# 42jaylonw/shifu

Measured on AMD Instinct MI355X. Metric: env-steps/sec (whole node), A1 12-dof 4096 envs/GPU, higher is better.
Workload: dtype f32

## Files before the change

shifu_amd/csrc/shf_a1_chain.hip:

```cpp
#include <hip/hip_runtime.h>

#include "shf_chain.h"
#include "shf_chain_hard.h"

template <int G, bool TW, bool SELF = false>
__global__ __launch_bounds__(256, (G == 32 ? 2 : 1)) void k_a1_chain(A1Args A) { a1_chain_step_body<G, A1Chain, TW, SELF>(A); }

#ifndef SHF_WR_FUSED
#define SHF_WR_FUSED 8
#endif
#ifndef SHF_WR_HOOK
#define SHF_WR_HOOK 0
#endif
template <bool TW, bool SELF>
__global__ __launch_bounds__(256, 2) void k_a1_chain_pgs(A1Args A) { a1_chain_step_body<32, A1Chain, TW, SELF, true, 8, false, SHF_WR_FUSED>(A); }
template <bool TW, bool SELF>
__global__ __launch_bounds__(256, 2) void k_a1_chain_pgs16(A1Args A) { a1_chain_step_body<32, A1Chain, TW, SELF, true, 16>(A); }
template <bool TW, bool SELF>
__global__ __launch_bounds__(256, 2) void k_a1_chain_tgs(A1Args A) { a1_chain_step_body<32, A1Chain, TW, SELF, true, 8, true, SHF_WR_FUSED>(A); }
template <bool TW, bool SELF>
__global__ __launch_bounds__(256, 2) void k_a1_chain_tgs16(A1Args A) { a1_chain_step_body<32, A1Chain, TW, SELF, true, 16, true>(A); }
#define SHF_PICK4(K, warped, self) ((self) ? ((warped) ? reinterpret_cast<const void*>(K<true, true>) : reinterpret_cast<const void*>(K<false, true>)) \
                                           : ((warped) ? reinterpret_cast<const void*>(K<true, false>) : reinterpret_cast<const void*>(K<false, false>)))
const void* shf_a1_chain_pgs_kernel(bool warped, bool self, bool k16, bool tgs) {
  if (tgs) return k16 ? SHF_PICK4(k_a1_chain_tgs16, warped, self) : SHF_PICK4(k_a1_chain_tgs, warped, self);
  return k16 ? SHF_PICK4(k_a1_chain_pgs16, warped, self) : SHF_PICK4(k_a1_chain_pgs, warped, self);
}
int shf_a1_chain_pgs_max_contacts(void) { return 16; }

template <bool TW, bool SELF, int KC, bool TGS>
DEV void sim_step_chain_pgs_body(const SimArgs& A) {
  extern __shared__ __attribute__((aligned(16))) float smem[];
  typedef A1Chain CD;
  constexpr int G = 32, nb = CD::NB, nd = CD::ND, NR = (CD::NEV + G - 1) / G;
  const int es = threadIdx.x / G, l = threadIdx.x % G;
  const int e = blockIdx.x * (256 / G) + es;
  stage_block<CHAIN_MODEL_BYTES>(A.model, smem);
  __syncthreads();
  const ShfModel* m = reinterpret_cast<const ShfModel*>(smem);
  if (e >= A.n) return;
  ChainLds L = chain_lds_carve<CD>(smem + CHAIN_MODEL_WORDS + es * chain_lds_words<CD>(0, SELF));
  const float* dof = A.dof + (size_t)e * nd * 2;
  const float* root = A.root + (size_t)e * 13;
  for (int i = l; i < 2 * nd; i += G) L.dofb[(i >> 1) * DOF_STRIDE + (i & 1)] = dof[i];
  if (l < 13) L.root[l] = root[l];
  GROUP_SYNC();
  StepCtx C;
  C.m = m; C.sp = A.sp; C.terr.t = A.terr; C.terr.h = A.heights; C.scene = nullptr;
  C.dropped = env_dropped(A.dropped, A.sp, e);
  C.mscale = A.mscale ? A.mscale + (size_t)e * nb : nullptr;
  const float mu = A.friction ? A.friction[e] : 1.0f;
  const int dl = l < nd ? l : 0;
  DofLane X = {L.dofb[dl * DOF_STRIDE], L.dofb[dl * DOF_STRIDE + 1], (A.effort && l < nd) ? A.effort[(size_t)e * nd + l] : 0.0f,
               (A.pos_tgt && l < nd) ? A.pos_tgt[(size_t)e * nd + l] : 0.0f, (A.vel_tgt && l < nd) ? A.vel_tgt[(size_t)e * nd + l] : 0.0f};
  ChainPoints<NR> LP;
  chain_points_load<G>(m, CD::NEV, l, C.sp.contact_offset + C.sp.rest_offset, LP);
  const RowLane RL = row_lane_load<CD>(l);
  chain_substep_hard<G, CD, TW, SELF, KC, TGS, (KC == 8 ? SHF_WR_HOOK : 0)>(C, L, l, X, LP, RL, A.body_force ? A.body_force + (size_t)e * nb * 3 : nullptr, mu, L.xch);
  if (l < nd) {
    A.dof[((size_t)e * nd + l) * 2] = X.q;
    A.dof[((size_t)e * nd + l) * 2 + 1] = X.qd;
  }
  if (l < 13) A.root[(size_t)e * 13 + l] = L.root[l];
  for (int i = l; i < 3 * nb; i += G) A.contact[(size_t)e * nb * 3 + i] = L.xch[i];
}
template <bool TW, bool SELF>
__global__ __launch_bounds__(256, 2) void k_sim_step_chain_pgs(SimArgs A) { sim_step_chain_pgs_body<TW, SELF, 8, false>(A); }
template <bool TW, bool SELF>
__global__ __launch_bounds__(256, 2) void k_sim_step_chain_pgs16(SimArgs A) { sim_step_chain_pgs_body<TW, SELF, 16, false>(A); }
template <bool TW, bool SELF>
__global__ __launch_bounds__(256, 2) void k_sim_step_chain_tgs(SimArgs A) { sim_step_chain_pgs_body<TW, SELF, 8, true>(A); }
template <bool TW, bool SELF>
__global__ __launch_bounds__(256, 2) void k_sim_step_chain_tgs16(SimArgs A) { sim_step_chain_pgs_body<TW, SELF, 16, true>(A); }
const void* shf_sim_step_chain_pgs_kernel(bool warped, bool self, bool k16, bool tgs) {
  if (tgs) return k16 ? SHF_PICK4(k_sim_step_chain_tgs16, warped, self) : SHF_PICK4(k_sim_step_chain_tgs, warped, self);
  return k16 ? SHF_PICK4(k_sim_step_chain_pgs16, warped, self) : SHF_PICK4(k_sim_step_chain_pgs, warped, self);
}
size_t shf_sim_step_chain_pgs_lds_bytes(bool self) { return ((size_t)CHAIN_MODEL_WORDS + 8 * (size_t)chain_lds_words<A1Chain>(0, self)) * 4; }

bool shf_a1_chain_matches(const ShfModel& m) { return A1Chain::matches(m); }
size_t shf_a1_chain_lds_bytes(int G, int nobs, bool self) {
  const int epb = 256 / G;
  return ((size_t)CHAIN_MODEL_WORDS + TASK_WORDS + STATS_LDS_WORDS + (size_t)epb * chain_lds_words<A1Chain>(SCR_OBS + nobs, self)) * 4;
}
const void* shf_a1_chain_kernel(int G, bool warped, bool self) {
  if (self) {
    if (G != 32) return nullptr;
    return warped ? reinterpret_cast<const void*>(k_a1_chain<32, true, true>) : reinterpret_cast<const void*>(k_a1_chain<32, false, true>);
  }
  switch (G) {
    case 16: return warped ? reinterpret_cast<const void*>(k_a1_chain<16, true>) : reinterpret_cast<const void*>(k_a1_chain<16, false>);
    case 32: return warped ? reinterpret_cast<const void*>(k_a1_chain<32, true>) : reinterpret_cast<const void*>(k_a1_chain<32, false>);
    default: return nullptr;
  }
}
#ifdef SHF_PHASE_CLOCK
int shf_a1_chain_phase_cycles(unsigned long long* out, int n, int reset) {
  unsigned long long h[48];
  if (hipMemcpyFromSymbol(h, HIP_SYMBOL(g_phase_cycles), sizeof h) != hipSuccess) return 1;
  for (int k = 0; k < n && k < 48; k++) out[k] = h[k];
  if (reset) {
    unsigned long long z[48] = {};
    if (hipMemcpyToSymbol(HIP_SYMBOL(g_phase_cycles), z, sizeof z) != hipSuccess) return 1;
  }
  return 0;
}
int shf_a1_chain_phase_waves(unsigned long long* out, int reset) {
  if (hipMemcpyFromSymbol(out, HIP_SYMBOL(g_phase_wave), sizeof(g_phase_wave)) != hipSuccess) return 1;
  if (reset) {
    void* p = nullptr;
    if (hipGetSymbolAddress(&p, HIP_SYMBOL(g_phase_wave)) != hipSuccess || hipMemset(p, 0, sizeof(g_phase_wave)) != hipSuccess) return 1;
// ... 5 lines not shown
```

shifu_amd/csrc/shf_chain.h:

```cpp
#pragma once
#include "shf_task.h"
#include "shf_link.h"

template <int NCH_, int NLK_, int NP_, int NEV_>
struct ChainDims {
  static constexpr int NCH = NCH_, NLK = NLK_, NB = 1 + NCH_ * (NLK_ + 1), ND = NCH_ * NLK_, NPC = NP_;
  static constexpr int NEV = NEV_;
  static constexpr int MAXPT = 9;
  static_assert(NEV_ >= NP_ && NEV_ <= 128, "evaluation slots: two 64-bit ballot words");
  DEV static constexpr int body(int c, int k) { return 1 + c * (NLK_ + 1) + k; }
  static bool matches(const ShfModel& m) {
    if (m.nb != NB || m.nd != ND || m.np != NPC || m.fixed_base || m.jtype[0] != SHF_JOINT_ROOT) return false;
    if (m.child_count[0] != NCH || m.nlevels != NLK) return false;
    if ((m.neval > 0 ? m.neval : m.np) != NEV) return false;
    int occupied = 0;
    for (int s = 0; s < NEV; s++) {
      const int i = m.pt_eval[s];
      if (i == -1) continue;
      if (i < 0 || i >= NPC || m.pt_slot[i] != s) return false;
      occupied++;
    }
    if (occupied != NPC) return false;
    for (int b = 0; b < NB; b++) {
      const int n = m.pt_count[b], i0 = m.pt_start[b];
      if (n > MAXPT) return false;
      if (n == 0 || m.dyn[b] != b) continue;
      const int s0 = m.pt_slot[i0];
      for (int j = 0; j < n; j++)
        if (m.pt_slot[i0 + j] != s0 + j) return false;
      if ((s0 >> 5) != ((s0 + n - 1) >> 5)) return false;
    }
    for (int c = 0; c < NCH; c++) {
      if (m.child_list[m.child_start[0] + c] != 1 + c * (NLK + 1)) return false;
      for (int k = 0; k <= NLK; k++) {
        const int b = 1 + c * (NLK + 1) + k;
        if (m.parent[b] != (k == 0 ? 0 : b - 1)) return false;
        if (k < NLK) {
          if (m.jtype[b] != SHF_JOINT_REVOLUTE || m.dof[b] != c * NLK + k || m.dyn[b] != b || m.level[b] != k + 1) return false;
          if (m.child_count[b] != (k < NLK - 1 ? 1 : 0)) return false;
          if (k < NLK - 1 && m.child_list[m.child_start[b]] != b + 1) return false;
        } else {
          if (m.jtype[b] != SHF_JOINT_WELD || m.dyn[b] != b - 1 || m.dof[b] != -1) return false;
        }
      }
    }
    return true;
  }
};
typedef ChainDims<4, 3, 76, 88> A1Chain;

#define JREC_STRIDE 16
#define JREC_QD 9
#define JREC_T0 12
#define JREC_DE 13
#define JREC_S 0
#define JREC_C 6
#define CHAIN_MODEL_BYTES ((int)offsetof(ShfModel, link_collide))
#define CHAIN_MODEL_WORDS ((CHAIN_MODEL_BYTES / 4 + 3) & ~3)
static_assert(CHAIN_MODEL_BYTES % 16 == 0, "stage_block copies 16-byte words");
template <class CD>
__host__ __device__ inline int chain_lds_words(int min_tail, bool self = false) {
  int tail = (CD::NPC + (self ? SHF_MAX_SELF_CONTACTS : 0)) * PT_STRIDE;
  if (tail < min_tail) tail = min_tail;
  const int w = CD::NB * POSE_STRIDE + ((CD::NB * 6 + 3) & ~3) + (CD::ND + 1) * XCH_STRIDE + CD::ND * JREC_STRIDE +
                ((CD::ND * DOF_STRIDE + 3) & ~3) + root_words(1) + tail;
  return (w + 3) & ~3;
}
struct ChainLds : EnvLds {
  float* jrec;
  float* xroot;
};
template <class CD>
DEV ChainLds chain_lds_carve(float* base) {
  static_assert(CD::ND * XCH_STRIDE >= 3 * CD::NB, "the exchange slots double as the contact-force staging");
  ChainLds L;
  L.pose = base;
  L.acc = L.pose + CD::NB * POSE_STRIDE;
  L.xch = L.acc + ((CD::NB * 6 + 3) & ~3);
  L.xroot = L.xch + CD::ND * XCH_STRIDE;
  L.jrec = L.xroot + XCH_STRIDE;
  L.dofb = L.jrec + CD::ND * JREC_STRIDE;
  L.root = L.dofb + ((CD::ND * DOF_STRIDE + 3) & ~3);
  L.pt = L.root + root_words(1);
  return L;
}

DEV void chain_ext_force(const float* F, const float* com, const float* Rw, const float* p, float* pA) {
  if (F[0] == 0.0f && F[1] == 0.0f && F[2] == 0.0f) return;
  float cw[3], t[3];
  mv3(Rw, com, cw);
#pragma unroll
  for (int k = 0; k < 3; k++) cw[k] += p[k];
  cross3(cw, F, t);
#pragma unroll
  for (int k = 0; k < 3; k++) { pA[k] -= t[k]; pA[3 + k] -= F[k]; }
}

DEV void chain_dof_effort(const StepCtx& C, int d, float q, float qd, float tau_cmd, float* t0o, float* deo, float tq = 0.0f, float tv_in = 0.0f) {
  const ShfModel* m = C.m;
  const float dt = C.sp.dt;
  float t0 = 0.0f, de = m->armature[d];
  const int mode = m->drive_mode[d];
  if (mode == SHF_DOF_MODE_EFFORT) {
    t0 = tau_cmd;
  } else if (mode == SHF_DOF_MODE_POS || mode == SHF_DOF_MODE_VEL) {
    float kp = mode == SHF_DOF_MODE_POS ? m->kp[d] : 0.0f, kd = m->kd[d];
    const float tv = mode == SHF_DOF_MODE_VEL ? tv_in : 0.0f;
    const float est = fmaf(kp, tq - q, kd * (tv - qd));
    const float lim = m->effort[d];
    if (lim > 0.0f && fabsf(est) > lim) { const float sc = lim / fabsf(est); kp *= sc; kd *= sc; }
    const float bj = fmaf(dt, kp, kd);
    t0 = fmaf(kp, tq - q, fmaf(kd, tv, -(bj * qd)));
    de = fmaf(dt, bj, de);
  }
  const float jd = m->damping[d];
  if (jd > 0.0f) { t0 = fmaf(-jd, qd, t0); de = fmaf(dt, jd, de); }
  const float lo = m->lower[d], up = m->upper[d];
  const float viol = q < lo ? lo - q : (q > up ? up - q : 0.0f);
  if (viol != 0.0f) {
    const float bl = fmaf(dt, C.sp.limit_k, C.sp.limit_d);
    t0 = fmaf(C.sp.limit_k, viol, fmaf(-bl, qd, t0));
    de = fmaf(dt, bl, de);
  }
  *t0o = t0; *deo = de;
}

template <int NR>
struct ChainPoints {
  int idx[NR];
  int body[NR];
  float pos[NR][3], rad[NR], thr[NR];
};
template <int G, int NR>
DEV void chain_points_load(const ShfModel* m, int nev, int l, float offset, ChainPoints<NR>& P) {
#pragma unroll
  for (int k = 0; k < NR; k++) {
    const int s = l + k * G;
    const int e = s < nev ? m->pt_eval[s] : -1;
    const int i = e < 0 ? 0 : e;
    P.idx[k] = e;
    P.body[k] = m->pt_body[i];
    P.rad[k] = m->pt_radius[i];
    P.thr[k] = (offset + P.rad[k]) * 1.01f + 1e-6f;
#pragma unroll
    for (int j = 0; j < 3; j++) P.pos[k][j] = m->pt_pos[i][j];
  }
}

DEV void terrain_height_gradient(const TerrainDev& T, float x, float y, float* h, float* gxo, float* gyo) {
  if (T.t.rows == 0) { *h = 0.0f; *gxo = 0.0f; *gyo = 0.0f; return; }
  float inv = 1.0f / T.t.hscale;
  float fx = (x + T.t.border) * inv, fy = (y + T.t.border) * inv;
  float fi = rclampf(floorf(fx), 0.0f, (float)(T.t.rows - 2)), fj = rclampf(floorf(fy), 0.0f, (float)(T.t.cols - 2));
  int i = (int)fi, j = (int)fj;
  float u = rclampf(fx - fi, 0.0f, 1.0f), v = rclampf(fy - fj, 0.0f, 1.0f);
  float vs = T.t.vscale;
  const int16_t* row0 = T.h + (size_t)i * T.t.cols + j;
  const int16_t* row1 = row0 + T.t.cols;
  float h00 = (float)row0[0] * vs, h10 = (float)row1[0] * vs, h01 = (float)row0[1] * vs, h11 = (float)row1[1] * vs;
  const bool lo = u + v <= 1.0f;
  float gx = (lo ? h10 : h11) - (lo ? h00 : h01);
  float gy = (lo ? h01 : h11) - (lo ? h00 : h10);
  *h = fmaf(lo ? v : 1.0f - v, lo ? gy : -gy, fmaf(lo ? u : 1.0f - u, lo ? gx : -gx, lo ? h00 : h11));
  *gxo = gx * inv; *gyo = gy * inv;
}
DEV void terrain_normal_from_gradient(const TerrainDev& T, float gx, float gy, float* n) {
  if (T.t.rows == 0) { n[0] = 0.0f; n[1] = 0.0f; n[2] = 1.0f; return; }
  const float nz = rsqrt_spec(fmaf(gy, gy, fmaf(gx, gx, 1.0f)));
  n[0] = -gx * nz; n[1] = -gy * nz; n[2] = nz;
}

struct SlotBits {
  unsigned long long w[2];
  DEV bool test(int s) const { return ((s < 64 ? w[0] >> s : w[1] >> (s - 64)) & 1ull) != 0ull; }
  DEV unsigned field(int s0, int n) const {
    const unsigned long long ww = s0 < 64 ? w[0] : w[1];
    return (unsigned)(ww >> (s0 & 63)) & ((1u << n) - 1u);
  }
};
template <int MAXPT>
struct SlotList {
  unsigned long long list;
  int i0, n, s0;
  SlotBits mask;
  DEV int slot(int j) const { return (int)((list >> (7 * j)) & 127ull); }
};
template <int MAXPT>
DEV SlotList<MAXPT> slot_list_load(const ShfModel* m, int i0, int n) {
  static_assert(MAXPT * 7 <= 64, "packed slot list");
  SlotList<MAXPT> S;
  S.list = 0ull; S.i0 = i0; S.n = n; S.s0 = m->pt_slot[n > 0 ? i0 : 0]; S.mask.w[0] = 0ull; S.mask.w[1] = 0ull;
  int sl[MAXPT];
#pragma unroll
  for (int j = 0; j < MAXPT; j++) sl[j] = m->pt_slot[j < n ? i0 + j : 0];
#pragma unroll
  for (int j = 0; j < MAXPT; j++) {
    if (j < n) {
      const int s = sl[j];
      S.list |= (unsigned long long)s << (7 * j);
      if (s < 64) S.mask.w[0] |= 1ull << s; else S.mask.w[1] |= 1ull << (s - 64);
    }
  }
  return S;
}

struct DofLane {
  float q, qd, tau;
  float tq, tv;
};

struct RowLane {
  int c, i;
  bool on;
  int off[6];
};
template <class CD>
DEV RowLane row_lane_load(int l) {
// ... 52 lines not shown
    for (int k = 0; k < 3; k++) { vc[k] = L.root[10 + k]; vc[3 + k] = L.root[7 + k]; }
    if (isroot && !(ROWS && ischain)) {
      pose_store(L.pose, Rc, pc, vc);
    } else {
      const int b0 = CD::body(ci, 0);
#pragma unroll
      for (int k = 0; k < NLK; k++) {
        const int b = b0 + k;
        float* rec = L.jrec + (ci * NLK + k) * JREC_STRIDE;
        float Rl[9];
#pragma unroll
        for (int j = 0; j < 9; j++) Rl[j] = rec[j];
        if constexpr (ROWS) {
          float Sx[6], cx[6];
          chain_compose_link(m->tpos[b], m->axis[b], Rl, rec[JREC_QD], Rc, pc, vc, Sx, cx);
#pragma unroll
          for (int j = 0; j < 6; j++) { rec[JREC_S + j] = Sx[j]; rec[JREC_C + j] = cx[j]; }
        } else {
          chain_compose_link(m->tpos[b], m->axis[b], Rl, rec[JREC_QD], Rc, pc, vc, K[k].S, K[k].c);
        }
        pose_store(L.pose + b * POSE_STRIDE, Rc, pc, vc);
      }
      const int b = b0 + NLK;
      chain_kin_weld(m->tpos[b], m->trot[b], Rc, pc);
      pose_store(L.pose + b * POSE_STRIDE, Rc, pc, vc);
    }
  }
  GROUP_SYNC();
  PHASE_MARK(1);

  float IA[21], pA[6];
  if (isbody) {
    const float* pb = L.pose + myb * POSE_STRIDE;
    float Rb[9], pp[3], vb[6];
#pragma unroll
    for (int k = 0; k < 9; k++) Rb[k] = pb[k];
#pragma unroll
    for (int k = 0; k < 3; k++) pp[k] = pb[9 + k];
#pragma unroll
    for (int k = 0; k < 6; k++) vb[k] = pb[12 + k];
    {
      float mass = m->mass[myb], I6[6];
#pragma unroll
      for (int k = 0; k < 6; k++) I6[k] = m->inertia[myb][k];
      if (C.mscale) {
        const float s = C.mscale[myb];
        mass *= s;
#pragma unroll
        for (int k = 0; k < 6; k++) I6[k] *= s;
      }
      rigid_inertia_p(mass, m->com[myb], I6, Rb, pp, vb, IA, pA);
    }
    if (fext) {
      const float F[3] = {fext[3 * myb], fext[3 * myb + 1], fext[3 * myb + 2]};
      chain_ext_force(F, m->com[myb], Rb, pp, pA);
      if (islink && (lb % NLK) == NLK - 1) {
        const int bw = myb + 1;
        const float* pw = L.pose + bw * POSE_STRIDE;
        float Rw[9], pq[3];
#pragma unroll
        for (int k = 0; k < 9; k++) Rw[k] = pw[k];
#pragma unroll
        for (int k = 0; k < 3; k++) pq[k] = pw[9 + k];
        const float Fw[3] = {fext[3 * bw], fext[3 * bw + 1], fext[3 * bw + 2]};
        chain_ext_force(Fw, m->com[bw], Rw, pq, pA);
      }
    }
  }
  PHASE_MARK(2);

  const float kc = C.sp.contact_k, dc = C.sp.contact_d, veps = C.sp.friction_vel;
  const float beta = fmaf(kc, dt, dc);
  const float mu = 0.5f * (mu_shape + C.terr.t.friction);
  const ContactConsts KC = {dt, {g[0], g[1], g[2]}, kc, beta, mu, veps, C.sp.max_depen_vel, C.sp.contact_offset};
  SlotBits act = {{0ull, 0ull}};
  {
    float r[NR][3], gx[NR], gy[NR], dz[NR], n[3];
    bool near[NR];
    const float nzmin = TW ? 0.0f : C.terr.t.nz_min;
#pragma unroll
    for (int k = 0; k < NR; k++) {
      const float* pb = L.pose + P.body[k] * POSE_STRIDE;
      float Rb[9], h = 0.0f;
#pragma unroll
      for (int j = 0; j < 9; j++) Rb[j] = pb[j];
      mv3(Rb, P.pos[k], r[k]);
#pragma unroll
      for (int j = 0; j < 3; j++) r[k][j] += pb[9 + j];
      if constexpr (TW) {
        gx[k] = 0.0f; gy[k] = 0.0f; dz[k] = 0.0f;
        near[k] = P.idx[k] >= 0;
      } else {
        terrain_height_gradient(C.terr, L.root[0] + r[k][0], L.root[1] + r[k][1], &h, &gx[k], &gy[k]);
        dz[k] = L.root[2] + r[k][2] - h;
        near[k] = P.idx[k] >= 0 && !(dz[k] * nzmin >= P.thr[k]);
      }
    }
    const int lane0 = (int)(threadIdx.x & 63u) - l;
#pragma unroll
    for (int k = 0; k < NR; k++) {
      if (__ballot(near[k]) == 0ull) continue;
      float on = 0.0f;
      if (near[k]) {
        float phi;
        if constexpr (TW) {
          float h;
          terrain_query<true>(C.terr, L.root[0] + r[k][0], L.root[1] + r[k][1], &h, n);
          phi = fmaf(L.root[2] + r[k][2] - h, n[2], -P.rad[k]);
        } else {
          terrain_normal_from_gradient(C.terr, gx[k], gy[k], n);
          phi = fmaf(dz[k], n[2], -P.rad[k]);
        }
        if (phi < KC.offset)
          on = contact_point_response(KC, L.pose + P.body[k] * POSE_STRIDE, r[k], n, P.rad[k], phi, L.pt + P.idx[k] * PT_STRIDE);
      }
      const unsigned long long bits = (__ballot(on != 0.0f) >> lane0) & (G >= 64 ? ~0ull : ((1ull << (G & 63)) - 1ull));
      if (k * G < 64) act.w[0] |= bits << ((k * G) & 63); else act.w[1] |= bits << ((k * G - 64) & 63);
    }
  }
  int nself = 0;
  if constexpr (SELF) nself = self_contacts_eval<G>(C, L, l, CD::NPC, mu_shape);
  GROUP_SYNC();
  PHASE_MARK(3);

  if (isbody) {
    if constexpr (SPLIT) {
      unsigned bits = act.field(mine.s0, mine.n);
      while (bits) {
        const int j = __builtin_ctz(bits);
        bits &= bits - 1u;
        const float* o = L.pt + (mine.i0 + j) * PT_STRIDE;
        if (half == 0) contact_accumulate_half<0>(o, dt, IA, pA);
        else contact_accumulate_half<1>(o, dt, IA, pA);
      }
    } else if (((act.w[0] & mine.mask.w[0]) | (act.w[1] & mine.mask.w[1])) != 0ull) {
      for (int j = 0; j < mine.n; j++) {
        if (!act.test(mine.slot(j))) continue;
        contact_accumulate_p(L.pt + (mine.i0 + j) * PT_STRIDE, dt, IA, pA);
      }
    }
    if constexpr (SELF) {
      for (int k = 0; k < nself; k++) {
        const float* o = L.pt + (CD::NPC + k) * PT_STRIDE;
        const int p = (int)o[PT_ON] - 1;
        const int da = m->dyn[m->cap_body[m->pair_a[p]]], db = m->dyn[m->cap_body[m->pair_b[p]]];
        if (da != myb && db != myb) continue;
        const float ma = body_mass(C, da), mb = body_mass(C, db);
// ... 259 lines not shown
    joint_local_rotation(m->trot[b], m->axis[b], X.q, Rl);
#pragma unroll
    for (int k = 0; k < 9; k++) rec[k] = Rl[k];
    rec[9] = X.qd;
  }
  GROUP_SYNC();
  if (l < NCH || l == ND) {
    float Rc[9], pc[3] = {0.0f, 0.0f, 0.0f}, vc[6], S[6], c[6];
    quat_to_mat(L.root + 3, Rc);
#pragma unroll
    for (int k = 0; k < 3; k++) { vc[k] = L.root[10 + k]; vc[3 + k] = L.root[7 + k]; }
    if (l == ND) {
      pose_store(L.pose, Rc, pc, vc);
    } else {
      const int b0 = CD::body(l, 0);
#pragma unroll
      for (int k = 0; k < NLK; k++) {
        const float* rec = L.jrec + (l * NLK + k) * JREC_STRIDE;
        float Rl[9];
#pragma unroll
        for (int j = 0; j < 9; j++) Rl[j] = rec[j];
        chain_compose_link(m->tpos[b0 + k], m->axis[b0 + k], Rl, rec[9], Rc, pc, vc, S, c);
        pose_store(L.pose + (b0 + k) * POSE_STRIDE, Rc, pc, vc);
      }
      chain_kin_weld(m->tpos[b0 + NLK], m->trot[b0 + NLK], Rc, pc);
      pose_store(L.pose + (b0 + NLK) * POSE_STRIDE, Rc, pc, vc);
    }
  }
  GROUP_SYNC();
  for (int b = l; b < NB; b += G) {
    const float* pb = L.pose + b * POSE_STRIDE;
    float Rw[9], pp[3], v[6], t[3], q[4];
#pragma unroll
    for (int k = 0; k < 9; k++) Rw[k] = pb[k];
#pragma unroll
    for (int k = 0; k < 3; k++) pp[k] = pb[9 + k];
#pragma unroll
    for (int k = 0; k < 6; k++) v[k] = pb[12 + k];
    float* o = stage + 13 * b;
#pragma unroll
    for (int k = 0; k < 3; k++) o[k] = L.root[k] + pp[k];
    mat_to_quat(Rw, q);
#pragma unroll
    for (int k = 0; k < 4; k++) o[3 + k] = q[k];
    cross3(v, pp, t);
#pragma unroll
    for (int k = 0; k < 3; k++) { o[7 + k] = v[3 + k] + t[k]; o[10 + k] = v[k]; }
  }
  GROUP_SYNC();
}

template <int G, class CD, bool TW, bool SELF, int KC, bool TGS, int WR>
DEV void chain_substep_hard(const StepCtx& C, const ChainLds& L, int l, DofLane& X, const ChainPoints<(CD::NEV + G - 1) / G>& P,
                            const RowLane& RL, const float* fext, float mu_shape, float* contact_out);
template <int G, class CD, bool TW, bool SELF = false, bool HARD = false, int KC = 8, bool TGS = false, int WR = 0>
DEV void a1_chain_step_body(const A1Args& A) {
  extern __shared__ __attribute__((aligned(16))) float smem[];
  constexpr int NLK = CD::NLK, nb = CD::NB, nd = CD::ND, NR = (CD::NEV + G - 1) / G;
  PHASE_BEGIN();
  float* stats_lds = smem + CHAIN_MODEL_WORDS + TASK_WORDS;
  stats_block_init(stats_lds);
  const unsigned long long stats_step = stats_step_load(A.stats);
  const int epb = 256 / G, es = threadIdx.x / G, l = threadIdx.x % G;
  const int e = blockIdx.x * epb + es;
  const int n = A.S.n;
  constexpr int NW = (2 * nd + G - 1) / G;
  float pre_dof[NW], pre_root = 0.0f, pre_act = 0.0f;
#pragma unroll
  for (int k = 0; k < NW; k++) pre_dof[k] = 0.0f;
  static_assert(G >= 13 && G > nd, "one root word and one action per lane");
  if (e < n) {
#pragma unroll
    for (int k = 0; k < NW; k++)
      if (l + k * G < 2 * nd) pre_dof[k] = A.S.dof[(size_t)e * nd * 2 + l + k * G];
    if (l < 13) pre_root = A.S.root[(size_t)e * 13 + l];
    if (l < nd) pre_act = raw_action(A, e, l, nd, stats_step);
  }
  stage_block<(int)sizeof(ShfA1TaskParams)>(A.tp, smem + CHAIN_MODEL_WORDS);
  stage_block<CHAIN_MODEL_BYTES>(A.S.model, smem);
  __syncthreads();
  const ShfModel* m = reinterpret_cast<const ShfModel*>(smem);
  const ShfA1TaskParams& tp = *reinterpret_cast<const ShfA1TaskParams*>(smem + CHAIN_MODEL_WORDS);
  if (e >= n) return;
  const int H = tp.num_history, P = tp.num_height_points;
  const int nobs = 12 + 2 * nd + nd * H + P;
  const int env_words = chain_lds_words<CD>(SCR_OBS + nobs, SELF);
  ChainLds L = chain_lds_carve<CD>(smem + CHAIN_MODEL_WORDS + TASK_WORDS + STATS_LDS_WORDS + es * env_words);
  float* scr = L.pt;

#pragma unroll
  for (int k = 0; k < NW; k++) {
    const int i = l + k * G;
    if (i < 2 * nd) L.dofb[(i >> 1) * DOF_STRIDE + (i & 1)] = pre_dof[k];
  }
  if (l < 13) L.root[l] = pre_root;
  float act = 0.0f;
  if (l < nd) {
    act = rclampf(pre_act * tp.action_scale, -tp.clip_actions, tp.clip_actions);
    A.actions[(size_t)e * nd + l] = act;
  }
  GROUP_SYNC();

  if (l == 0) {
    const float gv[3] = {0.0f, 0.0f, -1.0f};
    float pg[3], blv[3], bav[3];
    quat_rotate_inverse(L.root + 3, L.root + 7, blv);
    quat_rotate_inverse(L.root + 3, L.root + 10, bav);
    quat_rotate_inverse(L.root + 3, gv, pg);
    float* o = A.base_vel + (size_t)e * 9;
#pragma unroll
    for (int k = 0; k < 3; k++) { o[k] = blv[k]; o[3 + k] = bav[k]; o[6 + k] = pg[k]; }
  }

  StepCtx C;
  C.m = m; C.sp = A.S.sp; C.terr.t = A.S.terr; C.terr.h = A.S.heights; C.scene = nullptr;
  if constexpr (HARD) C.dropped = env_dropped(A.S.dropped, A.S.sp, e);
  C.mscale = A.S.mscale ? A.S.mscale + (size_t)e * nb : nullptr;
  const float mu = A.S.friction[e];
  const int nsub = tp.decimation + (tp.extra_substep ? 1 : 0);
  const int dl = l < nd ? l : 0;
  DofLane X = {L.dofb[dl * DOF_STRIDE], L.dofb[dl * DOF_STRIDE + 1], 0.0f};
  const float pg_ = tp.p_gain[dl], dg_ = tp.d_gain[dl], q0_ = tp.default_dof_pos[dl], lim_ = m->effort[dl];
  ChainPoints<NR> LP;
  if constexpr (!(HARD && WR > 0)) chain_points_load<G>(m, CD::NEV, l, HARD ? C.sp.contact_offset + C.sp.rest_offset : C.sp.contact_offset, LP);
  const int lb = G >= 32 ? (l & 15) : l;
  const int mb = lb < nd ? CD::body(lb / NLK, lb % NLK) : 0;
  const SlotList<CD::MAXPT> mine = slot_list_load<CD::MAXPT>(m, m->pt_start[mb], (lb <= nd && l < 32) ? m->pt_count[mb] : 0);
  const RowLane RL = row_lane_load<CD>(l);
  PHASE_MARK(11);
  for (int it = 0; it < nsub; it++) {
    if (it < tp.decimation) {
      const float t = pg_ * (act + q0_ - X.q) - dg_ * X.qd;
      X.tau = rclampf(t, -lim_, lim_);
    }
    if constexpr (HARD)
      chain_substep_hard<G, CD, TW, SELF, KC, TGS, WR>(C, L, l, X, LP, RL, (it == tp.decimation) ? A.push + (size_t)e * nb * 3 : nullptr, mu,
                                    (it == nsub - 1) ? L.xch : nullptr);
    else
      chain_substep<G, CD, TW, SELF>(C, L, l, X, LP, mine, RL, (it == tp.decimation) ? A.push + (size_t)e * nb * 3 : nullptr, mu,
                                     (it == nsub - 1) ? L.xch : nullptr);
  }
  PHASE_RESET();
  if (l < nd) {
    float* D = L.dofb + l * DOF_STRIDE;
    D[0] = X.q; D[1] = X.qd; D[5] = X.tau;
    A.torques[(size_t)e * nd + l] = X.tau;
    scr[SCR_ACT + l] = act;
  }
  for (int i = l; i < 3 * nb; i += G) A.S.contact[(size_t)e * nb * 3 + i] = L.xch[i];
  for (int i = l; i < nd * H; i += G) scr[SCR_HIST + i] = A.history[(size_t)e * nd * H + i];
  PHASE_MARK(12);
  chain_body_states<G, CD>(m, L, l, X, scr + SCR_BODY);
  for (int i = l; i < 13 * nb; i += G) A.body_state[(size_t)e * nb * 13 + i] = scr[SCR_BODY + i];
  PHASE_RESET();
  a1_post_step<G>(A, m, tp, L, scr, e, l, stats_lds, stats_step);
}
```

shifu_amd/csrc/shf_chain_hard.h:

```cpp
#pragma once
#include "shf_chain.h"

#define UF_STRIDE 8
template <class CD, int KC>
struct HardTail {
  static constexpr int HC = 0, W = KC * HC_STRIDE, NEVP = (CD::NEV + 3) & ~3;
  static constexpr bool PACKED = KC > 8;
  static constexpr int WS = PACKED ? 9 : 10;
  static constexpr int NBLK = PACKED ? KC * (KC + 1) / 2 : KC * KC;
  static constexpr int NB0 = PACKED ? (CD::NPC * PT_STRIDE - W) / 9 : NBLK;
  static constexpr int UF = W, PHI = W, END = W + NB0 * WS;
  static constexpr int SPARE = CD::NB * POSE_STRIDE + ((CD::NB * 6 + 3) & ~3) + CD::ND * XCH_STRIDE;
  static_assert(NEVP + SHF_MAX_SELF_CONTACTS <= NB0 * WS && CD::ND * UF_STRIDE <= NB0 * WS, "the gap list / U, 1/D fit the response matrix's place");
  static_assert(!PACKED || (NBLK - NB0) * 9 <= SPARE, "the rest of the packed response matrix fits the pose / rate / exchange slots");
  static_assert(KC <= 16 && (W % 2) == 0, "owner lanes, 16-bit constraint masks; 8-byte aligned blocks");
};
template <class CD, int KC>
DEV float* hard_wblock(const ChainLds& L, float* tail, int i, int j) {
  typedef HardTail<CD, KC> T;
  if constexpr (T::PACKED) {
    const int b = ((j * (j + 1)) >> 1) + i;
    return b < T::NB0 ? tail + T::W + b * 9 : L.pose + (b - T::NB0) * 9;
  } else {
    return tail + T::W + (j * KC + i) * T::WS;
// ... 287 lines not shown
DEV void hard_cap_extract(int l, int lane0, bool on, int* key, int& skey) {
  constexpr int NQ = NR + (SELF ? 1 : 0);
  constexpr int NONE = (int)0x80000000;
  int m = key[0];
#pragma unroll
  for (int k = 1; k < NR; k++) m = max(m, key[k]);
  if constexpr (SELF) m = max(m, skey);
  m = hard_env_max(m);
  int p = LAST ? -1 : 0x7fffffff;
#pragma unroll
  for (int k = 0; k < NQ; k++) {
    const unsigned b = (unsigned)(__ballot((k < NR ? key[k < NR ? k : 0] : skey) == m) >> lane0);
    if constexpr (LAST) p = max(p, (int)((b ? (unsigned)__builtin_clz(b) : ~0u) ^ (unsigned)(k * G + G - 1)));
    else p = (int)min((unsigned)p, (b ? (unsigned)__builtin_ctz(b) : ~0u) | (unsigned)(k * G));
  }
  const int d = on ? p - l : -1;
#pragma unroll
  for (int k = 0; k < NR; k++) key[k] = d == k * G ? NONE : key[k];
  if constexpr (SELF) skey = d == NR * G ? NONE : skey;
}
template <int G, int NR, bool SELF>
DEV void hard_cap_select(int l, int lane0, int total, int kmax, const float* ph, bool* cand, float sph, bool& scand) {
  static_assert(G == 32 && (NR + 1) * G <= 128, "two envs per wavefront; the positions of an env's candidates");
  constexpr int NONE = (int)0x80000000;
  const int excess = total - kmax;
  const bool keep = excess > kmax;
  int key[NR], skey = NONE;
#pragma unroll
  for (int k = 0; k < NR; k++) {
    const int q = hard_gap_key(ph[k]);
    key[k] = cand[k] ? (keep ? -q : q) : NONE;
  }
  if constexpr (SELF) {
    const int q = hard_gap_key(sph);
    skey = scand ? (keep ? -q : q) : NONE;
  }
  int n = keep ? 0 : excess;
  while (__ballot(n > 0) != 0ull) {
    hard_cap_extract<G, NR, SELF, true>(l, lane0, n > 0, key, skey);
    n--;
  }
  n = keep ? kmax : 0;
  while (__ballot(n > 0) != 0ull) {
    hard_cap_extract<G, NR, SELF, false>(l, lane0, n > 0, key, skey);
    n--;
  }
#pragma unroll
  for (int k = 0; k < NR; k++) cand[k] = cand[k] && ((key[k] == NONE) == keep);
  if constexpr (SELF) scand = scand && ((skey == NONE) == keep);
}

template <int G, class CD, bool TW, bool SELF, int KC, bool TGS, int WR>
DEV void chain_substep_hard(const StepCtx& C, const ChainLds& L, int l, DofLane& X, const ChainPoints<(CD::NEV + G - 1) / G>& PIN,
                            const RowLane& RL, const float* fext, float mu_shape, float* contact_out) {
  static_assert(G == 32, "the velocity-level solve is written for two envs per wavefront");
  constexpr int NCH = CD::NCH, NLK = CD::NLK, NB = CD::NB, ND = CD::ND, NR = (CD::NEV + G - 1) / G;
  typedef HardTail<CD, KC> T;
  static_assert(T::END <= CD::NPC * PT_STRIDE, "the solve's LDS fits the contact-slot region");
  static_assert((KC == 8 || KC == 16) && KC <= G / 2 + 8 && ND < 16, "owner lanes; a lane per column of the response matrix, in one or two passes");
  static_assert(WR >= 0 && WR <= KC && (WR == 0 || !T::PACKED), "the register row is the KC = 8 layout's");
  constexpr bool PIPE = WR > 0 && !SELF;
  constexpr bool SPLIT4 = WR > 0;
  constexpr bool CAPREG = !(SELF && (KC > 8 || (WR > 0 && TGS)));
  constexpr bool DROPATOM = WR > 0 && !TGS;
  const ShfModel* m = C.m;
  const float dt = C.sp.dt, idt = 1.0f / dt;
  const float gon = (float)m->gravity_on;
  const float g[3] = {C.sp.gravity[0] * gon, C.sp.gravity[1] * gon, C.sp.gravity[2] * gon};
  float* tail = L.pt;
  const int lb = l & 15;
  const int half = (l >> 4) & 1;
  const bool isdof = l < ND, isroot = l == ND;
  const bool ischain = (l & 7) == 0 && (l >> 3) < NCH;
  const int ci = l >> 3;
  const bool isbody = lb <= ND;
  const bool islink = isbody && lb < ND;
  const int myb = lb < ND ? CD::body(lb / NLK, lb % NLK) : 0;
  const int lane0 = (int)(threadIdx.x & 63u) - l;
  PHASE_BEGIN();
  ChainPoints<NR> PL;
  if constexpr (WR > 0) chain_points_load<G>(C.m, CD::NEV, l, C.sp.contact_offset + C.sp.rest_offset, PL);
  const ChainPoints<NR>& P = WR > 0 ? PL : PIN;

  if (isdof) {
    float* rec = L.jrec + l * JREC_STRIDE;
    float Rl[9], t0, de;
    chain_dof_effort(C, l, X.q, X.qd, X.tau, &t0, &de, X.tq, X.tv);
    joint_local_rotation(m->trot[myb], m->axis[myb], X.q, Rl);
#pragma unroll
    for (int k = 0; k < 9; k++) rec[k] = Rl[k];
    rec[JREC_QD] = X.qd; rec[JREC_T0] = t0; rec[JREC_DE] = de;
  }
  GROUP_SYNC();
  PHASE_MARK(0);

  if (ischain || isroot) {
    float Rc[9], pc[3] = {0.0f, 0.0f, 0.0f}, vc[6];
    quat_to_mat(L.root + 3, Rc);
#pragma unroll
    for (int k = 0; k < 3; k++) { vc[k] = L.root[10 + k]; vc[3 + k] = L.root[7 + k]; }
    if (isroot && !ischain) {
      pose_store(L.pose, Rc, pc, vc);
    } else {
      const int b0 = CD::body(ci, 0);
#pragma unroll
      for (int k = 0; k < NLK; k++) {
        const int b = b0 + k;
        float* rec = L.jrec + (ci * NLK + k) * JREC_STRIDE;
        float Rl[9], Sx[6], cx[6];
#pragma unroll
        for (int j = 0; j < 9; j++) Rl[j] = rec[j];
        chain_compose_link(m->tpos[b], m->axis[b], Rl, rec[JREC_QD], Rc, pc, vc, Sx, cx);
#pragma unroll
        for (int j = 0; j < 6; j++) { rec[JREC_S + j] = Sx[j]; rec[JREC_C + j] = cx[j]; }
        pose_store(L.pose + b * POSE_STRIDE, Rc, pc, vc);
      }
      const int b = b0 + NLK;
      chain_kin_weld(m->tpos[b], m->trot[b], Rc, pc);
      pose_store(L.pose + b * POSE_STRIDE, Rc, pc, vc);
    }
  }
  GROUP_SYNC();
  PHASE_MARK(1);

  if (isbody) {
    float IA[21], pA[6];
    const float* pb = L.pose + myb * POSE_STRIDE;
    float Rb[9], pp[3], vb[6];
#pragma unroll
    for (int k = 0; k < 9; k++) Rb[k] = pb[k];
#pragma unroll
    for (int k = 0; k < 3; k++) pp[k] = pb[9 + k];
#pragma unroll
    for (int k = 0; k < 6; k++) vb[k] = pb[12 + k];
    {
      float mass = m->mass[myb], I6[6];
#pragma unroll
      for (int k = 0; k < 6; k++) I6[k] = m->inertia[myb][k];
      if (C.mscale) {
        const float s = C.mscale[myb];
        mass *= s;
#pragma unroll
        for (int k = 0; k < 6; k++) I6[k] *= s;
      }
      rigid_inertia_p(mass, m->com[myb], I6, Rb, pp, vb, IA, pA);
    }
    if (fext) {
      const float F[3] = {fext[3 * myb], fext[3 * myb + 1], fext[3 * myb + 2]};
      chain_ext_force(F, m->com[myb], Rb, pp, pA);
      if (islink && (lb % NLK) == NLK - 1) {
        const int bw = myb + 1;
        const float* pw = L.pose + bw * POSE_STRIDE;
        float Rw[9], pq[3];
#pragma unroll
        for (int k = 0; k < 9; k++) Rw[k] = pw[k];
#pragma unroll
        for (int k = 0; k < 3; k++) pq[k] = pw[9 + k];
        const float Fw[3] = {fext[3 * bw], fext[3 * bw + 1], fext[3 * bw + 2]};
        chain_ext_force(Fw, m->com[bw], Rw, pq, pA);
      }
    }
    float* o = (islink ? L.xch + lb * XCH_STRIDE : L.xroot);
    if (half == 0) {
#pragma unroll
      for (int j = 0; j < 11; j++) o[j] = IA[j];
    } else {
#pragma unroll
      for (int j = 11; j < 21; j++) o[j] = IA[j];
#pragma unroll
      for (int j = 0; j < 6; j++) o[21 + j] = pA[j];
    }
  }
  PHASE_MARK(2);

  const float rest = C.sp.rest_offset, offs = C.sp.contact_offset + rest;
  const float mu = 0.5f * (mu_shape + C.terr.t.friction);
  const int kmax = hard_kmax_of(C.sp, KC);
  SlotBits act = {{0ull, 0ull}};
  int K;
  {
    float r[NR][3], nn[NR][3], ph[NR], gx[NR], gy[NR], dz[NR];
    bool near[NR], cand[NR];
    const float nzmin = TW ? 0.0f : C.terr.t.nz_min;
#pragma unroll
    for (int k = 0; k < NR; k++) {
      const float* pb = L.pose + P.body[k] * POSE_STRIDE;
      float Rb[9], h = 0.0f;
#pragma unroll
      for (int j = 0; j < 9; j++) Rb[j] = pb[j];
      mv3(Rb, P.pos[k], r[k]);
#pragma unroll
      for (int j = 0; j < 3; j++) r[k][j] += pb[9 + j];
      if constexpr (TW) {
        gx[k] = 0.0f; gy[k] = 0.0f; dz[k] = 0.0f;
        near[k] = P.idx[k] >= 0;
      } else {
        terrain_height_gradient(C.terr, L.root[0] + r[k][0], L.root[1] + r[k][1], &h, &gx[k], &gy[k]);
        dz[k] = L.root[2] + r[k][2] - h;
        near[k] = P.idx[k] >= 0 && !(dz[k] * nzmin >= P.thr[k]);
      }
    }
#pragma unroll
    for (int k = 0; k < NR; k++) {
      cand[k] = false; ph[k] = 0.0f;
      if (__ballot(near[k]) == 0ull) continue;
      if (near[k]) {
        float phi;
        if constexpr (TW) {
          float h;
          terrain_query<true>(C.terr, L.root[0] + r[k][0], L.root[1] + r[k][1], &h, nn[k]);
          phi = fmaf(L.root[2] + r[k][2] - h, nn[k][2], -P.rad[k]);
        } else {
          terrain_normal_from_gradient(C.terr, gx[k], gy[k], nn[k]);
          phi = fmaf(dz[k], nn[k][2], -P.rad[k]);
        }
        if (phi < offs) {
          cand[k] = true;
          ph[k] = phi - rest;
#pragma unroll
          for (int j = 0; j < 3; j++) r[k][j] = fmaf(-P.rad[k], nn[k][j], r[k][j]);
        }
      }
      const unsigned long long bits = (__ballot(cand[k]) >> lane0) & ((1ull << G) - 1ull);
      if (k * G < 64) act.w[0] |= bits << ((k * G) & 63); else act.w[1] |= bits << ((k * G - 64) & 63);
    }
    int nself = 0;
    if constexpr (SELF) nself = self_contacts_eval<G>(C, L, l, CD::NPC, mu_shape);
    if constexpr (SELF) GROUP_SYNC();
    const float* sslot = L.pt + (CD::NPC + (l < nself ? l : 0)) * PT_STRIDE;
    bool scand = SELF && l < nself;
    const float sph = scand ? sslot[PT_F] : 0.0f;
    const int npts = __popcll(act.w[0]) + __popcll(act.w[1]);
    int total = npts + nself;
    contact_hist_count(C, l, total);
    unsigned smask = nself >= 32 ? ~0u : ((1u << nself) - 1u);
    PHASE_MARK(30);
    if (__ballot(total > kmax) != 0ull) {
      if constexpr (CAPREG) {
        hard_cap_select<G, NR, SELF>(l, lane0, total, kmax, ph, cand, sph, scand);
      } else {
        float* lp = tail + T::PHI;
        int pos[NR];
#pragma unroll
        for (int k = 0; k < NR; k++) {
          const int sl = l + k * G;
          pos[k] = sl < 64 ? __popcll(act.w[0] & ((1ull << sl) - 1ull)) : __popcll(act.w[0]) + __popcll(act.w[1] & ((1ull << (sl - 64)) - 1ull));
          if (cand[k]) lp[pos[k]] = ph[k];
        }
        const int spos = npts + l;
        if (scand) lp[spos] = sph;
        if (l < 4) lp[total + l] = 3.0e38f;
        GROUP_SYNC();
        if (total > kmax) {
          int rank[NR], srank = 0;
#pragma unroll
          for (int k = 0; k < NR; k++) rank[k] = 0;
          for (int j4 = 0; j4 < total; j4 += 4) {
            const float4 pj4 = *reinterpret_cast<const float4*>(lp + j4);
            const float pj[4] = {pj4.x, pj4.y, pj4.z, pj4.w};
#pragma unroll
            for (int e = 0; e < 4; e++) {
#pragma unroll
              for (int k = 0; k < NR; k++) rank[k] += (pj[e] < ph[k] || (pj[e] == ph[k] && j4 + e < pos[k])) ? 1 : 0;
              if constexpr (SELF) srank += (pj[e] < sph || (pj[e] == sph && j4 + e < spos)) ? 1 : 0;
            }
          }
#pragma unroll
          for (int k = 0; k < NR; k++) cand[k] = cand[k] && rank[k] < kmax;
          if constexpr (SELF) scand = scand && srank < kmax;
        }
      }
      if (total > kmax && l == 0 && C.dropped) {
        if constexpr (DROPATOM) __hip_atomic_fetch_add(C.dropped, total - kmax, __ATOMIC_RELAXED, __HIP_MEMORY_SCOPE_AGENT);
        else *C.dropped += total - kmax;
      }
      act.w[0] = 0ull; act.w[1] = 0ull;
#pragma unroll
      for (int k = 0; k < NR; k++) {
        const unsigned long long bits = (__ballot(cand[k]) >> lane0) & ((1ull << G) - 1ull);
        if (k * G < 64) act.w[0] |= bits << ((k * G) & 63); else act.w[1] |= bits << ((k * G - 64) & 63);
      }
      smask = (unsigned)((__ballot(scand) >> lane0) & ((1ull << G) - 1ull));
      total = total > kmax ? kmax : total;
      if constexpr (!CAPREG) GROUP_SYNC();
    }
    PHASE_MARK(31);
    K = total;
    const int nps = __popcll(act.w[0]) + __popcll(act.w[1]);
    if (SELF && scand) {
      float* h = tail + T::HC + (nps + __popc(smask & ((1u << l) - 1u))) * HC_STRIDE;
      const int pr = (int)sslot[PT_ON] - 1;
      const int ba = m->cap_body[m->pair_a[pr]], bb = m->cap_body[m->pair_b[pr]];
#pragma unroll
      for (int j = 0; j < 3; j++) { h[HC_R + j] = sslot[PT_R + j]; h[HC_N + j] = sslot[PT_N + j]; }
      h[HC_PHI] = sph; h[HC_MU] = sslot[PT_F + 1];
      h[HC_BODY] = __int_as_float(m->dyn[ba]); h[HC_REP] = __int_as_float(ba);
      h[HC_BODYB] = __int_as_float(m->dyn[bb]); h[HC_REPB] = __int_as_float(bb);
      const float ns[3] = {sslot[PT_N], sslot[PT_N + 1], sslot[PT_N + 2]};
      hard_frame(ns, h + HC_T1, h + HC_T2);
    }
#pragma unroll
    for (int k = 0; k < NR; k++) {
      if (!cand[k]) continue;
      const int s = l + k * G;
      const int idx = s < 64 ? __popcll(act.w[0] & ((1ull << s) - 1ull)) : __popcll(act.w[0]) + __popcll(act.w[1] & ((1ull << (s - 64)) - 1ull));
      float* h = tail + T::HC + idx * HC_STRIDE;
#pragma unroll
      for (int j = 0; j < 3; j++) { h[HC_R + j] = r[k][j]; h[HC_N + j] = nn[k][j]; }
      h[HC_PHI] = ph[k]; h[HC_MU] = mu;
      h[HC_BODY] = __int_as_float(m->dyn[P.body[k]]); h[HC_REP] = __int_as_float(P.body[k]);
      h[HC_BODYB] = __int_as_float(-1); h[HC_REPB] = __int_as_float(-1);
      hard_frame(nn[k], h + HC_T1, h + HC_T2);
    }
  }
  GROUP_SYNC();
  PHASE_MARK(3);

  float uk[NLK];
  if (RL.on) {
    float Ic[6], pc = 0.0f;
    float* sx = L.acc + RL.c * 12;
#pragma unroll
    for (int k = NLK - 1; k >= 0; k--) {
      const float* o = L.xch + (RL.c * NLK + k) * XCH_STRIDE;
      const float* rec = L.jrec + (RL.c * NLK + k) * JREC_STRIDE;
      float row[6], S[6], cc[6], plg[6], Wg[6], Ug[6];
#pragma unroll
// ... 498 lines not shown
```

Measured before the change: 27.52 million.

## Batch terrain height loads, hoist push-force loads, and accumulate drop counts in LDS

Terrain height and gradient lookups for all contact rows are now gathered in one batch, so the global int16 loads for every row are issued before any of them is used, giving more memory-level parallelism. The tip-body external force load is hoisted out of the branch so it is issued unconditionally. Dropped-contact counts in the non-TGS hard path are summed in a per-env LDS word with workgroup-scope atomics and flushed to the global counter once per step, replacing per-substep device-scope atomics. In exchange the batched lookup holds more live registers, and in the non-TGS hard path the global counter is updated once per step instead of once per substep.

```diff
diff --git a/shifu_amd/csrc/shf_a1_chain.hip b/shifu_amd/csrc/shf_a1_chain.hip
--- a/shifu_amd/csrc/shf_a1_chain.hip
+++ b/shifu_amd/csrc/shf_a1_chain.hip
@@ -56,7 +56,7 @@
   ChainPoints<NR> LP;
   chain_points_load<G>(m, CD::NEV, l, C.sp.contact_offset + C.sp.rest_offset, LP);
   const RowLane RL = row_lane_load<CD>(l);
-  chain_substep_hard<G, CD, TW, SELF, KC, TGS, (KC == 8 ? SHF_WR_HOOK : 0)>(C, L, l, X, LP, RL, A.body_force ? A.body_force + (size_t)e * nb * 3 : nullptr, mu, L.xch);
+  chain_substep_hard<G, CD, TW, SELF, KC, TGS, (KC == 8 ? SHF_WR_HOOK : 0)>(C, L, l, X, LP, RL, A.body_force ? A.body_force + (size_t)e * nb * 3 : nullptr, mu, L.xch, nullptr);
   if (l < nd) {
     A.dof[((size_t)e * nd + l) * 2] = X.q;
     A.dof[((size_t)e * nd + l) * 2 + 1] = X.qd;
diff --git a/shifu_amd/csrc/shf_chain.h b/shifu_amd/csrc/shf_chain.h
--- a/shifu_amd/csrc/shf_chain.h
+++ b/shifu_amd/csrc/shf_chain.h
@@ -69,6 +69,7 @@
 struct ChainLds : EnvLds {
   float* jrec;
   float* xroot;
+  int* drops;
 };
 template <class CD>
 DEV ChainLds chain_lds_carve(float* base) {
@@ -77,6 +78,8 @@
   L.pose = base;
   L.acc = L.pose + CD::NB * POSE_STRIDE;
   L.xch = L.acc + ((CD::NB * 6 + 3) & ~3);
+  static_assert(((CD::NB * 6) & 3) != 0, "a padding word behind the accelerations for the drop sum");
+  L.drops = reinterpret_cast<int*>(L.acc + CD::NB * 6);
   L.xroot = L.xch + CD::ND * XCH_STRIDE;
   L.jrec = L.xroot + XCH_STRIDE;
   L.dofb = L.jrec + CD::ND * JREC_STRIDE;
@@ -147,22 +150,39 @@
   }
 }
 
-DEV void terrain_height_gradient(const TerrainDev& T, float x, float y, float* h, float* gxo, float* gyo) {
-  if (T.t.rows == 0) { *h = 0.0f; *gxo = 0.0f; *gyo = 0.0f; return; }
-  float inv = 1.0f / T.t.hscale;
-  float fx = (x + T.t.border) * inv, fy = (y + T.t.border) * inv;
-  float fi = rclampf(floorf(fx), 0.0f, (float)(T.t.rows - 2)), fj = rclampf(floorf(fy), 0.0f, (float)(T.t.cols - 2));
-  int i = (int)fi, j = (int)fj;
-  float u = rclampf(fx - fi, 0.0f, 1.0f), v = rclampf(fy - fj, 0.0f, 1.0f);
-  float vs = T.t.vscale;
-  const int16_t* row0 = T.h + (size_t)i * T.t.cols + j;
-  const int16_t* row1 = row0 + T.t.cols;
-  float h00 = (float)row0[0] * vs, h10 = (float)row1[0] * vs, h01 = (float)row0[1] * vs, h11 = (float)row1[1] * vs;
-  const bool lo = u + v <= 1.0f;
-  float gx = (lo ? h10 : h11) - (lo ? h00 : h01);
-  float gy = (lo ? h01 : h11) - (lo ? h00 : h10);
-  *h = fmaf(lo ? v : 1.0f - v, lo ? gy : -gy, fmaf(lo ? u : 1.0f - u, lo ? gx : -gx, lo ? h00 : h11));
-  *gxo = gx * inv; *gyo = gy * inv;
+template <int NR>
+DEV void terrain_height_gradient_rows(const TerrainDev& T, const float (*x)[2], float* h, float* gxo, float* gyo) {
+  if (T.t.rows == 0) {
+#pragma unroll
+    for (int k = 0; k < NR; k++) { h[k] = 0.0f; gxo[k] = 0.0f; gyo[k] = 0.0f; }
+    return;
+  }
+  const float inv = 1.0f / T.t.hscale, vs = T.t.vscale;
+  const float imax = (float)(T.t.rows - 2), jmax = (float)(T.t.cols - 2);
+  float u[NR], v[NR];
+  const int16_t* row0[NR];
+#pragma unroll
+  for (int k = 0; k < NR; k++) {
+    const float fx = (x[k][0] + T.t.border) * inv, fy = (x[k][1] + T.t.border) * inv;
+    const float fi = rclampf(floorf(fx), 0.0f, imax), fj = rclampf(floorf(fy), 0.0f, jmax);
+    u[k] = rclampf(fx - fi, 0.0f, 1.0f); v[k] = rclampf(fy - fj, 0.0f, 1.0f);
+    row0[k] = T.h + (size_t)(int)fi * T.t.cols + (int)fj;
+  }
+  int16_t s[NR][4];
+#pragma unroll
+  for (int k = 0; k < NR; k++) {
+    const int16_t* row1 = row0[k] + T.t.cols;
+    s[k][0] = row0[k][0]; s[k][1] = row1[0]; s[k][2] = row0[k][1]; s[k][3] = row1[1];
+  }
+#pragma unroll
+  for (int k = 0; k < NR; k++) {
+    const float h00 = (float)s[k][0] * vs, h10 = (float)s[k][1] * vs, h01 = (float)s[k][2] * vs, h11 = (float)s[k][3] * vs;
+    const bool lo = u[k] + v[k] <= 1.0f;
+    const float gx = (lo ? h10 : h11) - (lo ? h00 : h01);
+    const float gy = (lo ? h01 : h11) - (lo ? h00 : h10);
+    h[k] = fmaf(lo ? v[k] : 1.0f - v[k], lo ? gy : -gy, fmaf(lo ? u[k] : 1.0f - u[k], lo ? gx : -gx, lo ? h00 : h11));
+    gxo[k] = gx * inv; gyo[k] = gy * inv;
+  }
 }
 DEV void terrain_normal_from_gradient(const TerrainDev& T, float gx, float gy, float* n) {
   if (T.t.rows == 0) { n[0] = 0.0f; n[1] = 0.0f; n[2] = 1.0f; return; }
@@ -321,17 +341,18 @@
       rigid_inertia_p(mass, m->com[myb], I6, Rb, pp, vb, IA, pA);
     }
     if (fext) {
+      const bool tip = islink && (lb % NLK) == NLK - 1;
+      const int bw = tip ? myb + 1 : myb;
       const float F[3] = {fext[3 * myb], fext[3 * myb + 1], fext[3 * myb + 2]};
+      const float Fw[3] = {fext[3 * bw], fext[3 * bw + 1], fext[3 * bw + 2]};
       chain_ext_force(F, m->com[myb], Rb, pp, pA);
-      if (islink && (lb % NLK) == NLK - 1) {
-        const int bw = myb + 1;
+      if (tip) {
         const float* pw = L.pose + bw * POSE_STRIDE;
         float Rw[9], pq[3];
 #pragma unroll
         for (int k = 0; k < 9; k++) Rw[k] = pw[k];
 #pragma unroll
         for (int k = 0; k < 3; k++) pq[k] = pw[9 + k];
-        const float Fw[3] = {fext[3 * bw], fext[3 * bw + 1], fext[3 * bw + 2]};
         chain_ext_force(Fw, m->com[bw], Rw, pq, pA);
       }
     }
@@ -350,7 +371,7 @@
 #pragma unroll
     for (int k = 0; k < NR; k++) {
       const float* pb = L.pose + P.body[k] * POSE_STRIDE;
-      float Rb[9], h = 0.0f;
+      float Rb[9];
 #pragma unroll
       for (int j = 0; j < 9; j++) Rb[j] = pb[j];
       mv3(Rb, P.pos[k], r[k]);
@@ -359,9 +380,16 @@
       if constexpr (TW) {
         gx[k] = 0.0f; gy[k] = 0.0f; dz[k] = 0.0f;
         near[k] = P.idx[k] >= 0;
-      } else {
-        terrain_height_gradient(C.terr, L.root[0] + r[k][0], L.root[1] + r[k][1], &h, &gx[k], &gy[k]);
-        dz[k] = L.root[2] + r[k][2] - h;
+      }
+    }
+    if constexpr (!TW) {
+      float xy[NR][2], h[NR];
+#pragma unroll
+      for (int k = 0; k < NR; k++) { xy[k][0] = L.root[0] + r[k][0]; xy[k][1] = L.root[1] + r[k][1]; }
+      terrain_height_gradient_rows<NR>(C.terr, xy, h, gx, gy);
+#pragma unroll
+      for (int k = 0; k < NR; k++) {
+        dz[k] = L.root[2] + r[k][2] - h[k];
         near[k] = P.idx[k] >= 0 && !(dz[k] * nzmin >= P.thr[k]);
       }
     }
@@ -727,7 +755,7 @@
 
 template <int G, class CD, bool TW, bool SELF, int KC, bool TGS, int WR>
 DEV void chain_substep_hard(const StepCtx& C, const ChainLds& L, int l, DofLane& X, const ChainPoints<(CD::NEV + G - 1) / G>& P,
-                            const RowLane& RL, const float* fext, float mu_shape, float* contact_out);
+                            const RowLane& RL, const float* fext, float mu_shape, float* contact_out, int* drops);
 template <int G, class CD, bool TW, bool SELF = false, bool HARD = false, int KC = 8, bool TGS = false, int WR = 0>
 DEV void a1_chain_step_body(const A1Args& A) {
   extern __shared__ __attribute__((aligned(16))) float smem[];
@@ -769,6 +797,8 @@
     if (i < 2 * nd) L.dofb[(i >> 1) * DOF_STRIDE + (i & 1)] = pre_dof[k];
   }
   if (l < 13) L.root[l] = pre_root;
+  constexpr bool DROPSUM = HARD && !TGS;
+  if (DROPSUM && l == 0) *L.drops = 0;
   float act = 0.0f;
   if (l < nd) {
     act = rclampf(pre_act * tp.action_scale, -tp.clip_actions, tp.clip_actions);
@@ -810,12 +840,18 @@
     }
     if constexpr (HARD)
       chain_substep_hard<G, CD, TW, SELF, KC, TGS, WR>(C, L, l, X, LP, RL, (it == tp.decimation) ? A.push + (size_t)e * nb * 3 : nullptr, mu,
-                                    (it == nsub - 1) ? L.xch : nullptr);
+                                    (it == nsub - 1) ? L.xch : nullptr, DROPSUM ? L.drops : nullptr);
     else
       chain_substep<G, CD, TW, SELF>(C, L, l, X, LP, mine, RL, (it == tp.decimation) ? A.push + (size_t)e * nb * 3 : nullptr, mu,
                                      (it == nsub - 1) ? L.xch : nullptr);
   }
   PHASE_RESET();
+  if constexpr (DROPSUM) {
+    if (l == 0 && C.dropped) {
+      const int d = *L.drops;
+      if (d != 0) __hip_atomic_fetch_add(C.dropped, d, __ATOMIC_RELAXED, __HIP_MEMORY_SCOPE_AGENT);
+    }
+  }
   if (l < nd) {
     float* D = L.dofb + l * DOF_STRIDE;
     D[0] = X.q; D[1] = X.qd; D[5] = X.tau;
diff --git a/shifu_amd/csrc/shf_chain_hard.h b/shifu_amd/csrc/shf_chain_hard.h
--- a/shifu_amd/csrc/shf_chain_hard.h
+++ b/shifu_amd/csrc/shf_chain_hard.h
@@ -363,7 +363,7 @@
 
 template <int G, class CD, bool TW, bool SELF, int KC, bool TGS, int WR>
 DEV void chain_substep_hard(const StepCtx& C, const ChainLds& L, int l, DofLane& X, const ChainPoints<(CD::NEV + G - 1) / G>& PIN,
-                            const RowLane& RL, const float* fext, float mu_shape, float* contact_out) {
+                            const RowLane& RL, const float* fext, float mu_shape, float* contact_out, int* drops) {
   static_assert(G == 32, "the velocity-level solve is written for two envs per wavefront");
   constexpr int NCH = CD::NCH, NLK = CD::NLK, NB = CD::NB, ND = CD::ND, NR = (CD::NEV + G - 1) / G;
   typedef HardTail<CD, KC> T;
@@ -373,7 +373,6 @@
   constexpr bool PIPE = WR > 0 && !SELF;
   constexpr bool SPLIT4 = WR > 0;
   constexpr bool CAPREG = !(SELF && (KC > 8 || (WR > 0 && TGS)));
-  constexpr bool DROPATOM = WR > 0 && !TGS;
   const ShfModel* m = C.m;
   const float dt = C.sp.dt, idt = 1.0f / dt;
   const float gon = (float)m->gravity_on;
@@ -457,17 +456,18 @@
       rigid_inertia_p(mass, m->com[myb], I6, Rb, pp, vb, IA, pA);
     }
     if (fext) {
+      const bool tip = islink && (lb % NLK) == NLK - 1;
+      const int bw = tip ? myb + 1 : myb;
       const float F[3] = {fext[3 * myb], fext[3 * myb + 1], fext[3 * myb + 2]};
+      const float Fw[3] = {fext[3 * bw], fext[3 * bw + 1], fext[3 * bw + 2]};
       chain_ext_force(F, m->com[myb], Rb, pp, pA);
-      if (islink && (lb % NLK) == NLK - 1) {
-        const int bw = myb + 1;
+      if (tip) {
         const float* pw = L.pose + bw * POSE_STRIDE;
         float Rw[9], pq[3];
 #pragma unroll
         for (int k = 0; k < 9; k++) Rw[k] = pw[k];
 #pragma unroll
         for (int k = 0; k < 3; k++) pq[k] = pw[9 + k];
-        const float Fw[3] = {fext[3 * bw], fext[3 * bw + 1], fext[3 * bw + 2]};
         chain_ext_force(Fw, m->com[bw], Rw, pq, pA);
       }
     }
@@ -496,7 +496,7 @@
 #pragma unroll
     for (int k = 0; k < NR; k++) {
       const float* pb = L.pose + P.body[k] * POSE_STRIDE;
-      float Rb[9], h = 0.0f;
+      float Rb[9];
 #pragma unroll
       for (int j = 0; j < 9; j++) Rb[j] = pb[j];
       mv3(Rb, P.pos[k], r[k]);
@@ -505,9 +505,16 @@
       if constexpr (TW) {
         gx[k] = 0.0f; gy[k] = 0.0f; dz[k] = 0.0f;
         near[k] = P.idx[k] >= 0;
-      } else {
-        terrain_height_gradient(C.terr, L.root[0] + r[k][0], L.root[1] + r[k][1], &h, &gx[k], &gy[k]);
-        dz[k] = L.root[2] + r[k][2] - h;
+      }
+    }
+    if constexpr (!TW) {
+      float xy[NR][2], h[NR];
+#pragma unroll
+      for (int k = 0; k < NR; k++) { xy[k][0] = L.root[0] + r[k][0]; xy[k][1] = L.root[1] + r[k][1]; }
+      terrain_height_gradient_rows<NR>(C.terr, xy, h, gx, gy);
+#pragma unroll
+      for (int k = 0; k < NR; k++) {
+        dz[k] = L.root[2] + r[k][2] - h[k];
         near[k] = P.idx[k] >= 0 && !(dz[k] * nzmin >= P.thr[k]);
       }
     }
@@ -581,9 +588,9 @@
           if constexpr (SELF) scand = scand && srank < kmax;
         }
       }
-      if (total > kmax && l == 0 && C.dropped) {
-        if constexpr (DROPATOM) __hip_atomic_fetch_add(C.dropped, total - kmax, __ATOMIC_RELAXED, __HIP_MEMORY_SCOPE_AGENT);
-        else *C.dropped += total - kmax;
+      if (total > kmax && l == 0) {
+        if (drops) __hip_atomic_fetch_add(drops, total - kmax, __ATOMIC_RELAXED, __HIP_MEMORY_SCOPE_WORKGROUP);
+        else if (C.dropped) *C.dropped += total - kmax;
       }
       act.w[0] = 0ull; act.w[1] = 0ull;
 #pragma unroll
```

After: 27.68 million, median of 6. Within noise of the previous version (+0.6%).
